# turian/inverse-audio-synthesis

Measured on AMD Instinct MI355X. Metric: audio-seconds rendered+lossed/sec (whole node), batch=128 4s@44.1kHz, higher is better.
Workload: dtype f32; 1 GPU; BASELINE configs[1]: torchsynth-style Voice render + PQMF(3) analysis + mel-L1 loss, batch 128 x 4 s @ 44100 Hz per GPU; batch_per_gpu=128, samples_per_voice=176400, launch=hipgraph, streams=5, pipelined=True

## Files before the change

### inverse-audio-synthesis_amd/csrc/voice_ctrl_kernels.hip

```cpp
#define IAS_CTL_NO_LIBM
#include "voice_math.h"
#include "wave_ops.h"
#include "voice_table.h"

#define CS_THREADS 256
#define CS_WAVES (CS_THREADS / 64)
#define CS_KERNEL __global__ __launch_bounds__(CS_THREADS) __attribute__((amdgpu_num_vgpr(28)))

__constant__ IasParamRange c_cs_table[IAS_NPARAMS] = IAS_PARAM_TABLE_INIT;
__device__ const double g_cs_tab[IAS_CTL_TAB_DOUBLES] = IAS_CTL_TAB_INIT;

__device__ __forceinline__ void cs_stage_table(double* s_tab) {
  for (int i = threadIdx.x; i < IAS_CTL_TAB_DOUBLES; i += CS_THREADS) s_tab[i] = g_cs_tab[i];
}
__device__ __forceinline__ float cs_mapped(const float* __restrict__ params01, int b, int idx, const double* s_tab) {
  const IasParamRange r = c_cs_table[idx];
  return ias_map_param(params01[(size_t)b * IAS_NPARAMS + idx], (float)r.lo, (float)r.span, (float)r.curve, r.symmetric, s_tab);
}
__device__ __forceinline__ int cs_adsr_base(int a) {
  switch (a) {
    case 0: return IAS_P_ADSR_1_ATTACK;
    case 1: return IAS_P_ADSR_2_ATTACK;
    case 2: return IAS_P_LFO_1_AMP_ADSR_ATTACK;
    case 3: return IAS_P_LFO_2_AMP_ADSR_ATTACK;
    case 4: return IAS_P_LFO_1_RATE_ADSR_ATTACK;
    default: return IAS_P_LFO_2_RATE_ADSR_ATTACK;
  }
}

CS_KERNEL void voice_env_slim_kernel(const float* __restrict__ params01, float* __restrict__ sig, int Tc, float control_rate) {
  __shared__ __attribute__((aligned(16))) double s_tab[IAS_CTL_TAB_DOUBLES];
  __shared__ float s_p[8];
  const int a = blockIdx.x, b = blockIdx.y, tid = threadIdx.x;
  cs_stage_table(s_tab);
  __syncthreads();
  if (tid < 5) s_p[tid] = cs_mapped(params01, b, cs_adsr_base(a) + tid, s_tab);
  if (tid == 5) s_p[5] = cs_mapped(params01, b, IAS_P_KEYBOARD_DURATION, s_tab);
  __syncthreads();
  IasAdsr e;
  e.attack = s_p[0]; e.decay = s_p[1]; e.sustain = s_p[2]; e.release = s_p[3]; e.alpha = s_p[4];
  const float note_on = s_p[5], eps = (float)IAS_EPS;
  if (tid == 0) s_p[6] = ias_adsr_heads(e, note_on, control_rate, eps, s_tab).decay_head;
  if (tid == 64) s_p[7] = ias_adsr_heads(e, note_on, control_rate, eps, s_tab).release_head;
  __syncthreads();
  IasAdsrHeads heads;
  heads.decay_head = s_p[6]; heads.release_head = s_p[7];
  float* out = sig + ((size_t)b * 8 + a) * Tc;
  for (int t = tid; t < Tc; t += CS_THREADS) out[t] = ias_adsr_headed(t, e, note_on, control_rate, eps, heads, s_tab);
}

CS_KERNEL void voice_lfo_slim_kernel(const float* __restrict__ params01, float* __restrict__ sig,
                                     float* __restrict__ dbg ,
                                     int Tc, float control_rate) {
  extern __shared__ __attribute__((aligned(16))) double cs_smem[];
  double* s_tab = cs_smem;
  double* s_sum = s_tab + IAS_CTL_TAB_DOUBLES;
  __shared__ double s_wtot[CS_WAVES];
  __shared__ float s_q[8];
  __shared__ float s_mode[8];
  const int l = blockIdx.x, b = blockIdx.y, tid = threadIdx.x, lane = tid & 63, wave = tid >> 6;
  const int qbase = (l == 0) ? IAS_P_LFO_1_FREQUENCY : IAS_P_LFO_2_FREQUENCY;
  cs_stage_table(s_tab);
  __syncthreads();
  if (tid < 8) s_q[tid] = cs_mapped(params01, b, qbase + tid, s_tab);
  __syncthreads();
  if (tid < 5) s_mode[tid] = ias_pow_ctl(s_q[3 + tid], IAS_LFO_EXPONENT_F, s_tab);
  const float freq = s_q[0], depth = s_q[1], phi = s_q[2];
  const float* rate_env = sig + ((size_t)b * 8 + 4 + l) * Tc;
  const float* amp_env = sig + ((size_t)b * 8 + 2 + l) * Tc;

  const int per_wave = ((Tc + CS_WAVES - 1) / CS_WAVES + 63) / 64 * 64;
  const int t_begin = min(wave * per_wave, Tc), t_end = min(t_begin + per_wave, Tc);
  double carry = 0.0;
  for (int t0 = t_begin; t0 < t_end; t0 += 64) {
    const int t = t0 + lane;
    double inc = 0.0;
    if (t < t_end) inc = (double)ias_lfo_inc(freq, depth, rate_env[t], control_rate);
    const double sc = wave_incl_scan(inc, lane) + carry;
    carry = __shfl(sc, 63, 64);
    if (t < t_end) s_sum[t] = sc;
  }
  if (lane == 0) s_wtot[wave] = carry;
  __syncthreads();
  double base = 0.0;
  for (int w = 0; w < wave; ++w) base += s_wtot[w];
  float mode[5];
  {
    const float sm = (float)((double)s_mode[0] + (double)s_mode[1] + (double)s_mode[2] + (double)s_mode[3] + (double)s_mode[4]);
#pragma unroll
    for (int k = 0; k < 5; ++k) mode[k] = ias_div(s_mode[k], sm);
  }
  float* out = sig + ((size_t)b * 8 + 6 + l) * Tc;
  for (int t = t_begin + lane; t < t_end; t += 64) {
    const double ph = base + s_sum[t];
    const float arg = ias_add((float)ph, phi);
    const float o = ias_mul(ias_lfo_shape_mix(arg, mode, s_tab), amp_env[t]);
    out[t] = o;
    if (dbg != nullptr) {
      dbg[((size_t)b * 10 + 6 + l) * Tc + t] = arg;
      dbg[((size_t)b * 10 + 8 + l) * Tc + t] = o;
    }
  }
}

CS_KERNEL void voice_modmix_slim_kernel(const float* __restrict__ params01, const float* __restrict__ sig,
                                        float* __restrict__ ctrl, IasVoiceConst* __restrict__ vconst,
                                        float* __restrict__ dbg, int Tc) {
  __shared__ __attribute__((aligned(16))) double s_tab[IAS_CTL_TAB_DOUBLES];
  __shared__ float s_w[20];
  __shared__ float s_p[IAS_NPARAMS];
  const int b = blockIdx.y, tid = threadIdx.x;
  cs_stage_table(s_tab);
  __syncthreads();
  if (tid < 20) s_w[tid] = cs_mapped(params01, b, IAS_P_MOD_MATRIX_ADSR_1_TO_VCO_1_PITCH + tid, s_tab);
  if (blockIdx.x == 0 && tid >= 64 && tid < 64 + IAS_NPARAMS) s_p[tid - 64] = cs_mapped(params01, b, tid - 64, s_tab);
  __syncthreads();
  const float* sb = sig + (size_t)b * 8 * Tc;
  const int t = blockIdx.x * CS_THREADS + tid;
  if (t < Tc) {
    const float e0 = sb[t], e1 = sb[Tc + t], l0 = sb[6 * Tc + t], l1 = sb[7 * Tc + t];
    float* out = ctrl + (size_t)b * IAS_NCTRL * Tc;
#pragma unroll
    for (int j = 0; j < IAS_NCTRL; ++j)
      out[j * Tc + t] = ias_dot4_cr(s_w[j], s_w[5 + j], s_w[10 + j], s_w[15 + j], e0, e1, l0, l1);
    if (dbg != nullptr) {
#pragma unroll
      for (int r = 0; r < 6; ++r) dbg[((size_t)b * 10 + r) * Tc + t] = sb[r * Tc + t];
    }
  }
  if (blockIdx.x == 0 && tid == 0) {
    const float* p = s_p;
    const float midi_f0 = p[IAS_P_KEYBOARD_MIDI_F0];
    IasVoiceConst vc;
    vc.f0_1 = ias_add(midi_f0, p[IAS_P_VCO_1_TUNING]);
    vc.depth_1 = p[IAS_P_VCO_1_MOD_DEPTH];
    vc.phi_1 = p[IAS_P_VCO_1_INITIAL_PHASE];
    vc.f0_2 = ias_add(midi_f0, p[IAS_P_VCO_2_TUNING]);
    vc.depth_2 = p[IAS_P_VCO_2_MOD_DEPTH];
    vc.phi_2 = p[IAS_P_VCO_2_INITIAL_PHASE];
    vc.kpart = ias_partials_k(midi_f0, vc.depth_2, s_tab);
    vc.shape = p[IAS_P_VCO_2_SHAPE];
    vc.shape_gain = ias_sub(1.0f, ias_div(vc.shape, 2.0f));
    vc.lvl0 = p[IAS_P_MIXER_VCO_1];
    vc.lvl1 = p[IAS_P_MIXER_VCO_2];
    vc.lvl2 = p[IAS_P_MIXER_NOISE];
    vc.pad[0] = vc.pad[1] = vc.pad[2] = vc.pad[3] = 0.0f;
    vconst[b] = vc;
  }
}

bool ias_voice_control_slim_ok(int Tc, int control_rate) {
  return Tc <= 4096 && (double)Tc / (double)control_rate <= 600.0;
}
int ias_voice_control_slim_launch(const float* params01, float* ctrl, void* vconst, float* sig, float* dbg, int B, int Tc,
                                  int control_rate, hipStream_t stream) {
  const size_t lds = sizeof(double) * (IAS_CTL_TAB_DOUBLES + (size_t)Tc);
  hipLaunchKernelGGL(voice_env_slim_kernel, dim3(6, B), dim3(CS_THREADS), 0, stream, params01, sig, Tc, (float)control_rate);
  hipLaunchKernelGGL(voice_lfo_slim_kernel, dim3(2, B), dim3(CS_THREADS), lds, stream, params01, sig, dbg, Tc, (float)control_rate);
  hipLaunchKernelGGL(voice_modmix_slim_kernel, dim3((Tc + CS_THREADS - 1) / CS_THREADS, B), dim3(CS_THREADS), 0, stream, params01,
                     (const float*)sig, ctrl, (IasVoiceConst*)vconst, dbg, Tc);
  return hipGetLastError() == hipSuccess ? IAS_OK : IAS_ERR_LAUNCH;
}
```

### inverse-audio-synthesis_amd/csrc/voice_math.h

```cpp
#pragma once
#include "ias_common.h"
#include "voice_exp2_table.h"
#include "voice_ctrl_math.h"
#if !defined(__HIPCC__)
#include <algorithm>
using std::min;
using std::max;
#endif

#define IAS_PI_D 3.141592653589793
#define IAS_TWO_PI_D 6.283185307179586

#if defined(__clang__)
#pragma clang fp contract(off)
#endif
IAS_HD float ias_mul(float a, float b) { return a * b; }
IAS_HD float ias_add(float a, float b) { return a + b; }
IAS_HD float ias_sub(float a, float b) { return a - b; }
IAS_HD float ias_div(float a, float b) { return a / b; }
IAS_HD float ias_fma(float a, float b, float c) { return fmaf(a, b, c); }

IAS_HD float ias_pow_cr(float x, float a) { return (float)pow((double)x, (double)a); }
IAS_HD float ias_log2_cr(float x) { return (float)log2((double)x); }
IAS_HD float ias_log10_cr(float x) { return (float)log10((double)x); }
IAS_HD float ias_cos_cr(float x) { return (float)cos((double)x); }
IAS_HD float ias_exp2_slow_cr(float x) { return (float)exp2((double)x); }
#ifdef IAS_CTL_NO_LIBM
#define IAS_CTL_LIBM_IF(cond) if (false)
#else
#define IAS_CTL_LIBM_IF(cond) if (cond)
#endif
IAS_HD float ias_pow_ctl(float x, float a, const double* ctl) {
  IAS_CTL_LIBM_IF(ctl == nullptr || !ias_ctl_pow_in_domain(x, a)) return ias_pow_cr(x, a);
  if (!(x > 0.0f)) return x == 0.0f ? (a > 0.0f ? 0.0f : (a == 0.0f ? 1.0f : INFINITY)) : NAN;
  return (float)ias_ctl_pow(x, a, ctl);
}
IAS_HD float ias_cos_ctl(float x, const double* ctl) {
  IAS_CTL_LIBM_IF(ctl == nullptr || !ias_ctl_cos_in_domain(x)) return ias_cos_cr(x);
  return (float)ias_ctl_cos(x);
}
IAS_HD float ias_log2_ctl(float x, const double* ctl) {
  IAS_CTL_LIBM_IF(ctl == nullptr || !(x > 0.0f) || !(x < INFINITY)) return ias_log2_cr(x);
  if (!(x > 0.0f)) return x == 0.0f ? -INFINITY : NAN;
  return (float)ias_ctl_log2_value(x, ctl);
}
IAS_HD float ias_log10_ctl(float x, const double* ctl) {
  IAS_CTL_LIBM_IF(ctl == nullptr || !(x > 0.0f) || !(x < INFINITY) || fabsf(x - 1.0f) < 0.25f) return ias_log10_cr(x);
  return (float)ias_ctl_log10_value(x, ctl);
}
IAS_HD float ias_exp2_ctl(float v, const double* ctl) {
  IAS_CTL_LIBM_IF(ctl == nullptr) return ias_exp2_slow_cr(v);
  return (float)ias_ctl_exp2((double)v, 0.0, ctl);
}

IAS_HD float ias_exp2_cr(float t) {
  if (!(t > -160.0f)) return (t != t) ? t : 0.0f;
  if (t > 130.0f) return INFINITY;
  const float n = rintf(t);
  const double z = (double)(t - n) * 0.6931471805599453;
  double p = 1.6059043836821613e-10;
  p = fma(p, z, 2.08767569878681e-09);
  p = fma(p, z, 2.505210838544172e-08);
  p = fma(p, z, 2.755731922398589e-07);
  p = fma(p, z, 2.7557319223985893e-06);
  p = fma(p, z, 2.48015873015873e-05);
  p = fma(p, z, 0.0001984126984126984);
  p = fma(p, z, 0.001388888888888889);
  p = fma(p, z, 0.008333333333333333);
  p = fma(p, z, 0.041666666666666664);
  p = fma(p, z, 0.16666666666666666);
  p = fma(p, z, 0.5);
  p = fma(p, z, 1.0);
  p = fma(p, z, 1.0);
  return (float)ldexp(p, (int)n);
}

IAS_HD float ias_exp2_cr_fast(float t) {
  const float n = rintf(t);
  const double f = (double)(t - n);
  double p = 7.072587226569927e-09;
  p = fma(p, f, 1.0208690586037056e-07);
  p = fma(p, f, 1.3215442576793237e-06);
  p = fma(p, f, 1.5252657258547322e-05);
  p = fma(p, f, 0.00015403530441763784);
  p = fma(p, f, 0.001333355823016814);
  p = fma(p, f, 0.0096181291076068692);
  p = fma(p, f, 0.055504108664447695);
  p = fma(p, f, 0.24022650695910097);
  p = fma(p, f, 0.69314718055994995);
  p = fma(p, f, 1.0);
  return (float)ldexp(p, (int)n);
}

IAS_HD float ias_exp2_cr_tab(float t, const double* tab) {
  const float u = fmaf(t, 256.0f, 12582912.0f);
  const float mf = u - 12582912.0f;
  const float r = fmaf(mf, -0.00390625f, t);
  union { float f; int32_t i; } b;
  b.f = u;
  const double tv = tab[b.i - (0x4B400000 + IAS_EXP2_TAB_MIN)];
  const double rd = (double)r;
  double p = IAS_EXP2_C4;
  p = fma(p, rd, IAS_EXP2_C3);
  p = fma(p, rd, IAS_EXP2_C2);
  p = fma(p, rd, IAS_EXP2_C1);
  p = fma(p, rd, 1.0);
  return (float)(p * tv);
}

IAS_HD float ias_div_by_recip(float a, double recip) { return (float)((double)a * recip); }

IAS_HD float ias_div_fma(float a, float d, float r) {
  const float q0 = a * r;
  const float e = fmaf(-d, q0, a);
  return fmaf(e, r, q0);
}
IAS_HD int ias_div_fma_rate_ok(int sample_rate) {
  return sample_rate == 16000 || sample_rate == 22050 || sample_rate == 32000 || sample_rate == 44100 ||
         sample_rate == 48000 || sample_rate == 96000;
}

IAS_HD float ias_map_param(float u, float lo, float span, float curve, int symmetric, const double* ctl = nullptr) {
  if (!symmetric) {
    if (curve != 1.0f) u = ias_exp2_ctl(ias_div(ias_log2_ctl(u, ctl), curve), ctl);
    return ias_add(lo, ias_mul(span, u));
  }
  const float dist = ias_sub(ias_mul(2.0f, u), 1.0f);
  float v = dist;
  if (curve != 1.0f && dist != 0.0f) {
    const float mag = ias_exp2_ctl(ias_div(ias_log2_ctl(fabsf(dist), ctl), curve), ctl);
    v = dist < 0.0f ? -mag : mag;
  }
  return ias_add(lo, ias_mul(span, ias_add(v, 1.0f)));
}

IAS_HD float ias_ramp(int t, float duration, float start, int has_start, int inverse,
                      float alpha, float control_rate, float eps, const double* ctl = nullptr) {
  const float dur = ias_mul(duration, control_rate);
  float r = (float)t;
  if (has_start) r = ias_sub(r, ias_mul(start, control_rate));
  r = fmaxf(r, 0.0f);
  r = ias_add(ias_div(ias_add(r, eps), dur), eps);
  r = fminf(r, 1.0f);
  if (inverse && dur > 0.0f) r = ias_sub(1.0f, r);
  if (r == 1.0f || (r == 0.0f && alpha > 0.0f)) return r;
  return ias_pow_ctl(r, alpha, ctl);
}

struct IasAdsr { float attack, decay, sustain, release, alpha; };

IAS_HD float ias_ramp_headed(int t, float duration, float start, int inverse, float alpha, float control_rate,
                             float eps, float head, const double* ctl = nullptr) {
  if (ias_sub((float)t, ias_mul(start, control_rate)) <= 0.0f) return head;
  return ias_ramp(t, duration, start, 1, inverse, alpha, control_rate, eps, ctl);
}

struct IasAdsrHeads { float decay_head, release_head; };
IAS_HD IasAdsrHeads ias_adsr_heads(const IasAdsr& e, float note_on, float control_rate, float eps,
                                   const double* ctl = nullptr) {
  const float new_attack = fminf(e.attack, note_on);
  const float new_decay = fminf(fmaxf(ias_sub(note_on, e.attack), 0.0f), e.decay);
  IasAdsrHeads h;
  h.decay_head = ias_ramp(0, new_decay, new_attack, 1, 1, e.alpha, control_rate, eps, ctl);
  h.release_head = ias_ramp(0, e.release, note_on, 1, 1, e.alpha, control_rate, eps, ctl);
  return h;
}
IAS_HD float ias_adsr_headed(int t, const IasAdsr& e, float note_on, float control_rate, float eps,
                             const IasAdsrHeads& h, const double* ctl = nullptr) {
  const float new_attack = fminf(e.attack, note_on);
  const float new_decay = fminf(fmaxf(ias_sub(note_on, e.attack), 0.0f), e.decay);
  const float a = ias_ramp(t, new_attack, 0.0f, 0, 0, e.alpha, control_rate, eps, ctl);
  const float dr = ias_ramp_headed(t, new_decay, new_attack, 1, e.alpha, control_rate, eps, h.decay_head, ctl);
  const float d = ias_add(ias_mul(ias_sub(1.0f, e.sustain), dr), e.sustain);
  const float r = ias_ramp_headed(t, e.release, note_on, 1, e.alpha, control_rate, eps, h.release_head, ctl);
  return ias_mul(ias_mul(a, d), r);
}

IAS_HD float ias_adsr(int t, const IasAdsr& e, float note_on, float control_rate, float eps, const double* ctl = nullptr) {
  const float new_attack = fminf(e.attack, note_on);
  const float new_decay = fminf(fmaxf(ias_sub(note_on, e.attack), 0.0f), e.decay);
  const float a = ias_ramp(t, new_attack, 0.0f, 0, 0, e.alpha, control_rate, eps, ctl);
  const float dr = ias_ramp(t, new_decay, new_attack, 1, 1, e.alpha, control_rate, eps, ctl);
  const float d = ias_add(ias_mul(ias_sub(1.0f, e.sustain), dr), e.sustain);
  const float r = ias_ramp(t, e.release, note_on, 1, 1, e.alpha, control_rate, eps, ctl);
  return ias_mul(ias_mul(a, d), r);
}

IAS_HD float ias_lfo_inc(float freq, float depth, float rate_env, float control_rate) {
  const float fr = fmaxf(ias_add(freq, ias_mul(depth, rate_env)), 0.0f);
  return ias_div(ias_mul((float)IAS_TWO_PI_D, fr), control_rate);
}

IAS_HD float ias_remainder(float a, float b) {
  float m = fmodf(a, b);
  if (m != 0.0f && m < 0.0f) m = ias_add(m, b);
  return m;
}

IAS_HD float ias_remainder_2pi_ctl(float a, const double* ctl) {
  const float b = (float)IAS_TWO_PI_D;
  float m;
  m = ias_ctl_fmod(a, b, 1.0 / (double)(float)IAS_TWO_PI_D);
  IAS_CTL_LIBM_IF(ctl == nullptr || !ias_ctl_fmod_in_domain(a, b)) m = fmodf(a, b);
  if (m != 0.0f && m < 0.0f) m = ias_add(m, b);
  return m;
}

IAS_HD float ias_lfo_shape_mix(float arg, const float* mode, const double* ctl = nullptr) {
  const float two_pi = (float)IAS_TWO_PI_D;
  float c = ias_cos_ctl(ias_add(arg, (float)IAS_PI_D), ctl);
  float sq = (c > 0.0f) ? 1.0f : ((c < 0.0f) ? -1.0f : 0.0f);
  c = ias_div(ias_add(c, 1.0f), 2.0f);
  sq = ias_div(ias_add(sq, 1.0f), 2.0f);
  const float saw = ias_div(ias_remainder_2pi_ctl(arg, ctl), two_pi);
  const float rsaw = ias_sub(1.0f, saw);
  float tri = ias_mul(2.0f, saw);
  if (tri > 1.0f) tri = ias_sub(2.0f, tri);
  double o = (double)mode[0] * (double)c;
  o += (double)mode[1] * (double)tri;
  o += (double)mode[2] * (double)saw;
  o += (double)mode[3] * (double)rsaw;
  o += (double)mode[4] * (double)sq;
  return (float)o;
}

IAS_HD float ias_dot4_cr(float w0, float w1, float w2, float w3, float s0, float s1, float s2, float s3) {
  double o = (double)w0 * (double)s0;
  o += (double)w1 * (double)s1;
  o += (double)w2 * (double)s2;
  o += (double)w3 * (double)s3;
  return (float)o;
}

IAS_HD void ias_lfo_mode(const float* p5, float* mode, const double* ctl = nullptr) {
  float m[5];
  for (int k = 0; k < 5; ++k) m[k] = ias_pow_ctl(p5[k], IAS_LFO_EXPONENT_F, ctl);
  const float s = (float)((double)m[0] + (double)m[1] + (double)m[2] + (double)m[3] + (double)m[4]);
  for (int k = 0; k < 5; ++k) mode[k] = ias_div(m[k], s);
}

IAS_HD void ias_interp_pos(int j, float scale, int Tc, int& i0, int& i1, float& w0, float& w1) {
  const float real = ias_mul(scale, (float)j);
  int k = (int)floorf(real);
  if (k > Tc - 1) k = Tc - 1;
  i0 = k;
  i1 = k + (k < Tc - 1 ? 1 : 0);
  w1 = fminf(fmaxf(ias_sub(real, (float)k), 0.0f), 1.0f);
  w0 = ias_sub(1.0f, w1);
}
IAS_HD void ias_interp_pos_fast(int j, float scale, int Tc, int& i0, int& i1, float& w0, float& w1) {
  const float real = ias_mul(scale, (float)j);
  const int k = (int)real;
  i0 = k;
  i1 = min(k + 1, Tc - 1);
  w1 = ias_sub(real, (float)k);
  w0 = ias_sub(1.0f, w1);
}
IAS_HD float ias_lerp(float a, float b, float w0, float w1) { return fmaf(w0, a, ias_mul(w1, b)); }

IAS_HD float ias_midi_to_hz(float midi) {
  return ias_mul(440.0f, ias_exp2_cr(ias_div(ias_sub(midi, 69.0f), 12.0f)));
}

IAS_HD float ias_vco_inc(float f0, float depth, float pitch_mod, float sample_rate) {
  float c = ias_add(f0, ias_mul(depth, pitch_mod));
  c = fminf(fmaxf(c, 0.0f), 127.0f);
  return ias_div(ias_mul((float)IAS_TWO_PI_D, ias_midi_to_hz(c)), sample_rate);
}

IAS_HD float ias_vco_inc_fast(float f0, float depth, float pitch_mod, double inv_sample_rate) {
  float c = ias_add(f0, ias_mul(depth, pitch_mod));
  c = fminf(fmaxf(c, 0.0f), 127.0f);
  const float t = ias_div_by_recip(ias_sub(c, 69.0f), 1.0 / 12.0);
  const float hz = ias_mul(440.0f, ias_exp2_cr_fast(t));
  return ias_div_by_recip(ias_mul((float)IAS_TWO_PI_D, hz), inv_sample_rate);
}

IAS_HD float ias_partials_k(float midi_f0, float depth_2, const double* ctl = nullptr) {
  const float max_pitch = ias_add(midi_f0, fmaxf(depth_2, 0.0f));
  const float max_f0 = ias_midi_to_hz(max_pitch);
  const float partials = ias_div(12000.0f, ias_mul(max_f0, ias_log10_ctl(max_f0, ctl)));
  return ias_mul((float)IAS_PI_D, partials);
}

#if defined(__HIPCC__)
__device__ __forceinline__ void ias_sincos_dev(float a, float& s, float& c) {
  const double v = (double)a * 0.15915494309189535;
  const double r = v - rint(v);
  const double q = rint(r + r);
  const float r2 = (float)fma(q, -0.5, r);
  const float sg = ((int)q & 1) ? -1.0f : 1.0f;
  s = sg * __builtin_amdgcn_sinf(r2);
  c = sg * __builtin_amdgcn_cosf(r2);
}
__device__ __forceinline__ float ias_cos_dev(float a) {
  const double v = (double)a * 0.15915494309189535;
  return __builtin_amdgcn_cosf((float)(v - rint(v)));
}
__device__ __forceinline__ float ias_tanh_dev(float z) {
  const float t = __builtin_amdgcn_exp2f(-2.885390081777927f * fabsf(z));
  const float r = (1.0f - t) * __builtin_amdgcn_rcpf(1.0f + t);
  return z < 0.0f ? -r : r;
}
__device__ __forceinline__ float ias_mix_sample_dev(float arg1, float arg2, float amp1, float amp2, float ampn,
                                                    float noise, const IasVoiceConst& vc) {
  float s2, c2;
  ias_sincos_dev(arg2, s2, c2);
  const float v1 = ias_mul(ias_cos_dev(arg1), amp1);
  const float sq = ias_tanh_dev(ias_mul(ias_mul(vc.kpart, s2), 0.5f));
  const float v2 = ias_mul(ias_mul(ias_mul(vc.shape_gain, sq), ias_add(1.0f, ias_mul(vc.shape, c2))), amp2);
  const float nz = ias_mul(noise, ampn);
  float o = ias_mul(vc.lvl0, v1);
  o = ias_add(o, ias_mul(vc.lvl1, v2));
  o = ias_add(o, ias_mul(vc.lvl2, nz));
  return o;
}

#endif

IAS_HD float ias_mix_sample(float arg1, float arg2, float amp1, float amp2, float ampn,
                            float noise, const IasVoiceConst& vc) {
  const float v1 = ias_mul(cosf(arg1), amp1);
  const float sq = tanhf(ias_mul(ias_mul(vc.kpart, sinf(arg2)), 0.5f));
  const float v2 = ias_mul(ias_mul(ias_mul(vc.shape_gain, sq),
                                   ias_add(1.0f, ias_mul(vc.shape, cosf(arg2)))), amp2);
  const float nz = ias_mul(noise, ampn);
  float o = ias_mul(vc.lvl0, v1);
  o = ias_add(o, ias_mul(vc.lvl1, v2));
  o = ias_add(o, ias_mul(vc.lvl2, nz));
  return o;
}
```

Baseline: 3.269 million audio-s/s.

## Skip saturated ADSR ramp regions and restructure modmix as one block per voice

The envelope kernel now binary-searches the time boundaries where each attack, decay and release ramp is saturated or not yet started, then evaluates the costly pow only inside the active ranges and uses precomputed head and tail constants elsewhere. The modmix kernel switches to one block per batch item with a strided time loop. It no longer stages the double table in LDS and maps only the 31 needed parameters instead of all of them. This cuts per-sample transcendental work and redundant per-block table staging, at the risk of bit mismatches at region boundaries and less parallelism in modmix.

```diff
diff --git a/inverse-audio-synthesis_amd/csrc/voice_ctrl_kernels.hip b/inverse-audio-synthesis_amd/csrc/voice_ctrl_kernels.hip
--- a/inverse-audio-synthesis_amd/csrc/voice_ctrl_kernels.hip
+++ b/inverse-audio-synthesis_amd/csrc/voice_ctrl_kernels.hip
@@ -30,7 +30,8 @@
 
 CS_KERNEL void voice_env_slim_kernel(const float* __restrict__ params01, float* __restrict__ sig, int Tc, float control_rate) {
   __shared__ __attribute__((aligned(16))) double s_tab[IAS_CTL_TAB_DOUBLES];
-  __shared__ float s_p[8];
+  __shared__ float s_p[10];
+  __shared__ int s_bound[IAS_ADSR_NBOUND];
   const int a = blockIdx.x, b = blockIdx.y, tid = threadIdx.x;
   cs_stage_table(s_tab);
   __syncthreads();
@@ -40,13 +41,19 @@
   IasAdsr e;
   e.attack = s_p[0]; e.decay = s_p[1]; e.sustain = s_p[2]; e.release = s_p[3]; e.alpha = s_p[4];
   const float note_on = s_p[5], eps = (float)IAS_EPS;
+  const IasAdsrRamps g = ias_adsr_ramps(e, note_on, control_rate);
   if (tid == 0) s_p[6] = ias_adsr_heads(e, note_on, control_rate, eps, s_tab).decay_head;
   if (tid == 64) s_p[7] = ias_adsr_heads(e, note_on, control_rate, eps, s_tab).release_head;
+  if (tid >= 128 && tid < 128 + IAS_ADSR_NBOUND) s_bound[tid - 128] = ias_adsr_boundary(tid - 128, g, Tc, eps);
+  if (tid == 192) s_p[8] = ias_ramp_tail(g.dur_d, 1, e.alpha, s_tab);
+  if (tid == 193) s_p[9] = ias_ramp_tail(g.dur_r, 1, e.alpha, s_tab);
   __syncthreads();
-  IasAdsrHeads heads;
-  heads.decay_head = s_p[6]; heads.release_head = s_p[7];
+  IasAdsrFlats f;
+  f.d_head = s_p[6]; f.r_head = s_p[7]; f.d_tail = s_p[8]; f.r_tail = s_p[9];
+  IasAdsrRegions q;
+  q.a_sat = s_bound[0]; q.d_begin = s_bound[1]; q.d_sat = s_bound[2]; q.r_begin = s_bound[3]; q.r_sat = s_bound[4];
   float* out = sig + ((size_t)b * 8 + a) * Tc;
-  for (int t = tid; t < Tc; t += CS_THREADS) out[t] = ias_adsr_headed(t, e, note_on, control_rate, eps, heads, s_tab);
+  for (int t = tid; t < Tc; t += CS_THREADS) out[t] = ias_adsr_regional(t, e, g, q, f, eps, s_tab);
 }
 
 CS_KERNEL void voice_lfo_slim_kernel(const float* __restrict__ params01, float* __restrict__ sig,
@@ -103,47 +110,56 @@
   }
 }
 
+#define CS_NVC 11
+__constant__ int c_cs_vc_param[CS_NVC] = {IAS_P_KEYBOARD_MIDI_F0, IAS_P_VCO_1_TUNING, IAS_P_VCO_1_MOD_DEPTH, IAS_P_VCO_1_INITIAL_PHASE,
+                                          IAS_P_VCO_2_TUNING, IAS_P_VCO_2_MOD_DEPTH, IAS_P_VCO_2_INITIAL_PHASE, IAS_P_VCO_2_SHAPE,
+                                          IAS_P_MIXER_VCO_1, IAS_P_MIXER_VCO_2, IAS_P_MIXER_NOISE};
+
 CS_KERNEL void voice_modmix_slim_kernel(const float* __restrict__ params01, const float* __restrict__ sig,
                                         float* __restrict__ ctrl, IasVoiceConst* __restrict__ vconst,
                                         float* __restrict__ dbg, int Tc) {
-  __shared__ __attribute__((aligned(16))) double s_tab[IAS_CTL_TAB_DOUBLES];
-  __shared__ float s_w[20];
-  __shared__ float s_p[IAS_NPARAMS];
-  const int b = blockIdx.y, tid = threadIdx.x;
-  cs_stage_table(s_tab);
-  __syncthreads();
-  if (tid < 20) s_w[tid] = cs_mapped(params01, b, IAS_P_MOD_MATRIX_ADSR_1_TO_VCO_1_PITCH + tid, s_tab);
-  if (blockIdx.x == 0 && tid >= 64 && tid < 64 + IAS_NPARAMS) s_p[tid - 64] = cs_mapped(params01, b, tid - 64, s_tab);
+  __shared__ float s_w[20 + CS_NVC];
+  const int b = blockIdx.x, tid = threadIdx.x;
+  if (tid < 20 + CS_NVC)
+    s_w[tid] = cs_mapped(params01, b, tid < 20 ? IAS_P_MOD_MATRIX_ADSR_1_TO_VCO_1_PITCH + tid : c_cs_vc_param[tid - 20], g_cs_tab);
   __syncthreads();
   const float* sb = sig + (size_t)b * 8 * Tc;
-  const int t = blockIdx.x * CS_THREADS + tid;
-  if (t < Tc) {
-    const float e0 = sb[t], e1 = sb[Tc + t], l0 = sb[6 * Tc + t], l1 = sb[7 * Tc + t];
-    float* out = ctrl + (size_t)b * IAS_NCTRL * Tc;
+  float* out = ctrl + (size_t)b * IAS_NCTRL * Tc;
+  float* db = dbg != nullptr ? dbg + (size_t)b * 10 * Tc : nullptr;
+  const unsigned n = (unsigned)Tc;
+  float w[20];
 #pragma unroll
-    for (int j = 0; j < IAS_NCTRL; ++j)
-      out[j * Tc + t] = ias_dot4_cr(s_w[j], s_w[5 + j], s_w[10 + j], s_w[15 + j], e0, e1, l0, l1);
+  for (int i = 0; i < 20; ++i) w[i] = s_w[i];
+  for (unsigned t = tid; t < n; t += CS_THREADS) {
+#pragma unroll
+    for (int i = 0; i < 20; ++i) asm volatile("" : "+v"(w[i]));
+    const float e0 = sb[t], e1 = sb[n + t], l0 = sb[6 * n + t], l1 = sb[7 * n + t];
+#pragma unroll
+    for (unsigned j = 0; j < IAS_NCTRL; ++j)
+      out[j * n + t] = ias_dot4_cr(w[j], w[5 + j], w[10 + j], w[15 + j], e0, e1, l0, l1);
     if (dbg != nullptr) {
+      db[t] = e0;
+      db[n + t] = e1;
 #pragma unroll
-      for (int r = 0; r < 6; ++r) dbg[((size_t)b * 10 + r) * Tc + t] = sb[r * Tc + t];
+      for (unsigned r = 2; r < 6; ++r) db[r * n + t] = sb[r * n + t];
     }
   }
-  if (blockIdx.x == 0 && tid == 0) {
-    const float* p = s_p;
-    const float midi_f0 = p[IAS_P_KEYBOARD_MIDI_F0];
+  if (tid == 0) {
+    const float* p = s_w + 20;
+    const float midi_f0 = p[0];
     IasVoiceConst vc;
-    vc.f0_1 = ias_add(midi_f0, p[IAS_P_VCO_1_TUNING]);
-    vc.depth_1 = p[IAS_P_VCO_1_MOD_DEPTH];
-    vc.phi_1 = p[IAS_P_VCO_1_INITIAL_PHASE];
-    vc.f0_2 = ias_add(midi_f0, p[IAS_P_VCO_2_TUNING]);
-    vc.depth_2 = p[IAS_P_VCO_2_MOD_DEPTH];
-    vc.phi_2 = p[IAS_P_VCO_2_INITIAL_PHASE];
-    vc.kpart = ias_partials_k(midi_f0, vc.depth_2, s_tab);
-    vc.shape = p[IAS_P_VCO_2_SHAPE];
+    vc.f0_1 = ias_add(midi_f0, p[1]);
+    vc.depth_1 = p[2];
+    vc.phi_1 = p[3];
+    vc.f0_2 = ias_add(midi_f0, p[4]);
+    vc.depth_2 = p[5];
+    vc.phi_2 = p[6];
+    vc.kpart = ias_partials_k(midi_f0, vc.depth_2, g_cs_tab);
+    vc.shape = p[7];
     vc.shape_gain = ias_sub(1.0f, ias_div(vc.shape, 2.0f));
-    vc.lvl0 = p[IAS_P_MIXER_VCO_1];
-    vc.lvl1 = p[IAS_P_MIXER_VCO_2];
-    vc.lvl2 = p[IAS_P_MIXER_NOISE];
+    vc.lvl0 = p[8];
+    vc.lvl1 = p[9];
+    vc.lvl2 = p[10];
     vc.pad[0] = vc.pad[1] = vc.pad[2] = vc.pad[3] = 0.0f;
     vconst[b] = vc;
   }
@@ -157,7 +173,7 @@
   const size_t lds = sizeof(double) * (IAS_CTL_TAB_DOUBLES + (size_t)Tc);
   hipLaunchKernelGGL(voice_env_slim_kernel, dim3(6, B), dim3(CS_THREADS), 0, stream, params01, sig, Tc, (float)control_rate);
   hipLaunchKernelGGL(voice_lfo_slim_kernel, dim3(2, B), dim3(CS_THREADS), lds, stream, params01, sig, dbg, Tc, (float)control_rate);
-  hipLaunchKernelGGL(voice_modmix_slim_kernel, dim3((Tc + CS_THREADS - 1) / CS_THREADS, B), dim3(CS_THREADS), 0, stream, params01,
-                     (const float*)sig, ctrl, (IasVoiceConst*)vconst, dbg, Tc);
+  hipLaunchKernelGGL(voice_modmix_slim_kernel, dim3(B), dim3(CS_THREADS), 0, stream, params01, (const float*)sig, ctrl,
+                     (IasVoiceConst*)vconst, dbg, Tc);
   return hipGetLastError() == hipSuccess ? IAS_OK : IAS_ERR_LAUNCH;
 }
diff --git a/inverse-audio-synthesis_amd/csrc/voice_math.h b/inverse-audio-synthesis_amd/csrc/voice_math.h
--- a/inverse-audio-synthesis_amd/csrc/voice_math.h
+++ b/inverse-audio-synthesis_amd/csrc/voice_math.h
@@ -134,17 +134,23 @@
   return ias_add(lo, ias_mul(span, ias_add(v, 1.0f)));
 }
 
+IAS_HD float ias_ramp_pos(int t, float dur, float start_c, int has_start, float eps) {
+  float r = (float)t;
+  if (has_start) r = ias_sub(r, start_c);
+  r = fmaxf(r, 0.0f);
+  r = ias_add(ias_div(ias_add(r, eps), dur), eps);
+  return fminf(r, 1.0f);
+}
+IAS_HD float ias_ramp_finish(float r, float dur, int inverse, float alpha, const double* ctl = nullptr) {
+  if (inverse && dur > 0.0f) r = ias_sub(1.0f, r);
+  if (r == 1.0f || (r == 0.0f && alpha > 0.0f)) return r;
+  return ias_pow_ctl(r, alpha, ctl);
+}
 IAS_HD float ias_ramp(int t, float duration, float start, int has_start, int inverse,
                       float alpha, float control_rate, float eps, const double* ctl = nullptr) {
   const float dur = ias_mul(duration, control_rate);
-  float r = (float)t;
-  if (has_start) r = ias_sub(r, ias_mul(start, control_rate));
-  r = fmaxf(r, 0.0f);
-  r = ias_add(ias_div(ias_add(r, eps), dur), eps);
-  r = fminf(r, 1.0f);
-  if (inverse && dur > 0.0f) r = ias_sub(1.0f, r);
-  if (r == 1.0f || (r == 0.0f && alpha > 0.0f)) return r;
-  return ias_pow_ctl(r, alpha, ctl);
+  const float start_c = has_start ? ias_mul(start, control_rate) : 0.0f;
+  return ias_ramp_finish(ias_ramp_pos(t, dur, start_c, has_start, eps), dur, inverse, alpha, ctl);
 }
 
 struct IasAdsr { float attack, decay, sustain, release, alpha; };
@@ -183,6 +189,59 @@
   const float dr = ias_ramp(t, new_decay, new_attack, 1, 1, e.alpha, control_rate, eps, ctl);
   const float d = ias_add(ias_mul(ias_sub(1.0f, e.sustain), dr), e.sustain);
   const float r = ias_ramp(t, e.release, note_on, 1, 1, e.alpha, control_rate, eps, ctl);
+  return ias_mul(ias_mul(a, d), r);
+}
+
+struct IasAdsrRamps { float dur_a, dur_d, dur_r, start_d, start_r; };
+IAS_HD IasAdsrRamps ias_adsr_ramps(const IasAdsr& e, float note_on, float control_rate) {
+  const float new_attack = fminf(e.attack, note_on);
+  const float new_decay = fminf(fmaxf(ias_sub(note_on, e.attack), 0.0f), e.decay);
+  IasAdsrRamps g;
+  g.dur_a = ias_mul(new_attack, control_rate);
+  g.dur_d = ias_mul(new_decay, control_rate);
+  g.dur_r = ias_mul(e.release, control_rate);
+  g.start_d = ias_mul(new_attack, control_rate);
+  g.start_r = ias_mul(note_on, control_rate);
+  return g;
+}
+#define IAS_ADSR_NBOUND 5
+IAS_HD int ias_adsr_boundary(int k, const IasAdsrRamps& g, int Tc, float eps) {
+  const bool begin = (k == 1 || k == 3);
+  if (g.dur_a < 0.0f || g.dur_d < 0.0f || g.dur_r < 0.0f) return begin ? 0 : Tc;
+  const float dur = k == 0 ? g.dur_a : (k <= 2 ? g.dur_d : g.dur_r);
+  const float start_c = k == 0 ? 0.0f : (k <= 2 ? g.start_d : g.start_r);
+  int lo = 0, hi = Tc;
+  while (lo < hi) {
+    const int mid = (lo + hi) >> 1;
+    const bool p = begin ? !(ias_sub((float)mid, start_c) <= 0.0f)
+                         : ias_ramp_pos(mid, dur, start_c, k != 0, eps) == 1.0f;
+    if (p) hi = mid; else lo = mid + 1;
+  }
+  return lo;
+}
+struct IasAdsrRegions { int a_sat, d_begin, d_sat, r_begin, r_sat; };
+IAS_HD IasAdsrRegions ias_adsr_regions(const IasAdsrRamps& g, int Tc, float eps) {
+  IasAdsrRegions q;
+  q.a_sat = ias_adsr_boundary(0, g, Tc, eps);
+  q.d_begin = ias_adsr_boundary(1, g, Tc, eps);
+  q.d_sat = ias_adsr_boundary(2, g, Tc, eps);
+  q.r_begin = ias_adsr_boundary(3, g, Tc, eps);
+  q.r_sat = ias_adsr_boundary(4, g, Tc, eps);
+  return q;
+}
+IAS_HD float ias_ramp_tail(float dur, int inverse, float alpha, const double* ctl = nullptr) {
+  return ias_ramp_finish(1.0f, dur, inverse, alpha, ctl);
+}
+struct IasAdsrFlats { float d_head, d_tail, r_head, r_tail; };
+IAS_HD float ias_adsr_regional(int t, const IasAdsr& e, const IasAdsrRamps& g, const IasAdsrRegions& q, const IasAdsrFlats& f,
+                               float eps, const double* ctl = nullptr) {
+  float a = ias_ramp_tail(g.dur_a, 0, e.alpha, ctl);
+  if (t < q.a_sat) a = ias_ramp_finish(ias_ramp_pos(t, g.dur_a, 0.0f, 0, eps), g.dur_a, 0, e.alpha, ctl);
+  float dr = t < q.d_begin ? f.d_head : f.d_tail;
+  if (t >= q.d_begin && t < q.d_sat) dr = ias_ramp_finish(ias_ramp_pos(t, g.dur_d, g.start_d, 1, eps), g.dur_d, 1, e.alpha, ctl);
+  const float d = ias_add(ias_mul(ias_sub(1.0f, e.sustain), dr), e.sustain);
+  float r = t < q.r_begin ? f.r_head : f.r_tail;
+  if (t >= q.r_begin && t < q.r_sat) r = ias_ramp_finish(ias_ramp_pos(t, g.dur_r, g.start_r, 1, eps), g.dur_r, 1, e.alpha, ctl);
   return ias_mul(ias_mul(a, d), r);
 }
 
```

After: 3.270 million audio-s/s (median of 3 runs). About the same (+0.0%).
